# ShittyWizard/DiplomJourney

Measured on NVIDIA B200. Metric: candidate rollouts/s (MPC inner loop), higher is better.
Workload: dtype f32

## Files before the change

diplomjourney_b200/csrc/mpcb_handle.cuh:

```cuda
#pragma once
#include <string>
#include <vector>

#include "mpcb_types.cuh"

namespace mpcb {

struct DevBuf {
    void *p = nullptr;
    size_t cap = 0;
    cudaError_t ensure(size_t bytes) {
        if (bytes <= cap) return cudaSuccess;
        if (p) cudaFree(p);
        p = nullptr; cap = 0;
        size_t want = bytes + bytes / 4 + 256;
        cudaError_t e = cudaMalloc(&p, want);
        if (e == cudaSuccess) cap = want;
        return e;
    }
    void release() { if (p) cudaFree(p); p = nullptr; cap = 0; }
    template <typename T> T *as() { return reinterpret_cast<T *>(p); }
};

constexpr unsigned long long kSegCap = 1ULL << 22;
constexpr unsigned long long kTileBatch = 1ULL << 23;
constexpr unsigned long long kWideReduceSegs = 1ULL << 15;
constexpr unsigned long long kFrontierCap = 1ULL << 22;

}

struct mpcb_handle_s {
    int device = 0, sms = 148;
    cudaStream_t stream = nullptr;
    std::string err;
    bool have_grid = false, tables_ready = false;
    std::vector<double> hv, hb;
    double L = 0, delta_t = 0, v_min = 0, v_slow = 0;
    mpcb::GridTables g{};
    mpcb::DevBuf tab64, tab32, vtab, tab64_slow, vtab_slow, beta, leaf32, leaf32p, leaf32r, ctl32, ctl32_slow;
    mpcb::RowPairs row_ab{};
    double tol_scale = 1.0;
    int algo = MPCB_ALGO_AUTO;
    int refine = 1;
    int small_path = 1;
    int zero_copy = 1;
    int dump_direct = 0;
    int npt = 2;
    unsigned long long frontier_cap = mpcb::kFrontierCap;
    int subtree_cut = 2;
    int screen = 2;
    int prefilter = 1;
    int prune = 1;
    mpcb::DevBuf sp, segmin, worklist, misc, tau, bestJ, bestIdx, lock, ub, tile_list, reduce_scratch;
    mpcb::DevBuf in_state, in_target, in_origin, in_thr, in_flags, out_cost, out_index, out_traj, out_ctl, dump_rec, dump_j;
    mpcb::DevBuf cand, cand_J, cand_sel;
    mpcb::DevBuf node_list;
    unsigned node_cap = 1u << 15;
    unsigned cand_cap = 1u << 20;
    bool cand_auto = true;
    mpcb::DevBuf nccl_scratch;
    mpcb::DevBuf loop_log, loop_ticks, loop_status, loop_events, loop_final, loop_rng, loop_keys, small_in, small_out, fl_last, fl_k, fl_have, fl_flags, fl_count;
    void *pin_in = nullptr, *pin_out = nullptr;
    size_t pin_in_cap = 0, pin_out_cap = 0;
    mpcb_stats stats{};
};
```

diplomjourney_b200/csrc/mpcb_kernels.cu:

```cuda
#include <type_traits>

#include "mpcb_types.cuh"
#include "mpcb_bounds.cuh"
#include "mpcb_exact.cuh"

#ifndef MPCB_UNROLL2
#define MPCB_UNROLL2 8
#endif
#ifndef MPCB_UNROLL4
#define MPCB_UNROLL4 2
#endif
#ifndef MPCB_PN_CTA2
#define MPCB_PN_CTA2 512
#endif
#ifndef MPCB_UNROLL_ROWS
#define MPCB_UNROLL_ROWS 4
#endif
#ifndef MPCB_UNROLL_DIST
#define MPCB_UNROLL_DIST 7
#endif
#ifndef MPCB_UNROLL
#define MPCB_UNROLL 8
#endif

// ... 134 lines not shown
        walk_step_t<float>(t.x, t.y, t.z, t.w, xi, eta, psi, cp, sp);
    });
    return node_prefilter32(pf, xi, eta, psi, cp, sp) > __double2float_ru(bound + 8.0 * P.tol1);
}

__device__ __forceinline__ double node_lower_bound(const LaunchArgs &a, const SolveParams &P, const NodeFrame &f) {
    return lower_bound_from(a, P, f.u, f.w, f.Dp, f.nu, f.nw, 1.0, 0.0, f.ep, f.hp, f.base0, 1);
}

__device__ __forceinline__ double node_regs(const LaunchArgs &a, const NodeFrame &f, ParentRegs &pr, bool &near,
                                            double *base_direct) {
    pr.u = (float)f.u; pr.w = (float)f.w;
    pr.u2 = (float)(-2.0 * f.u); pr.w2 = (float)(-2.0 * f.w);
    const double dp_rem = split_distance(f.Dp, pr);
    pr.nu = (float)f.nu; pr.nw = (float)f.nw;
    pr.e2 = (float)(2.0 * f.ep); pr.h2 = (float)(2.0 * f.hp);
    near = !(f.Dp >= 4.0 * a.g.smax);
    if (base_direct) {
        pr.eh = 0.5f * pr.e2; pr.nhh = -0.5f * pr.h2;
        pr.u2s = (float)(-2.0 * kWd * kWd * f.u); pr.w2s = (float)(-2.0 * kWd * kWd * f.w);
        pr.D2s = (float)(kWd * kWd * (f.Dp * f.Dp));
        *base_direct = f.base0 - kWd * f.Dp - (double)pr.eh * (double)pr.eh - (double)pr.nhh * (double)pr.nhh;
    }
    return f.base0 + (near ? dp_rem : 0.0);
}

__device__ __forceinline__ double parent_setup(const LaunchArgs &a, const SolveParams &P,
                                               unsigned long long p, ParentRegs &pr, bool &near, bool &unmoved,
                                               double *lower_bound = nullptr, double *base_direct = nullptr) {
    NodeFrame f;
    node_frame(a, P, p, f);
    unmoved = f.unmoved;
    if (lower_bound) *lower_bound = node_lower_bound(a, P, f);
    return node_regs(a, f, pr, near, base_direct);
}

__device__ __forceinline__ bool cand_push(const LaunchArgs &a, long long n, long long j, double jrel) {
    if (!a.cand) return false;
    const unsigned slot = atomicAdd(a.cand_count, 1u);
    if (slot >= a.cand_cap) return false;
    Candidate c;
    c.j = j; c.jrel = jrel; c.n = (int)n; c.pad = 0;
    a.cand[slot] = c;
    return true;
}

__device__ __forceinline__ void take_candidate(const LaunchArgs &a, const SolveParams &P, long long n, long long j,
                                               double jrel32, double &bJ, long long &bj) {
    atomicAdd(a.counters + 1, 1ULL);
    if (cand_push(a, n, j, jrel32)) return;
    double J = a.refine ? exact_cost(a, P, j, nullptr, nullptr) : (P.Kbase + jrel32);
    lex_min(bJ, bj, J, j);
}

__device__ __forceinline__ void publish_best(const LaunchArgs &a, long long n, double bJ, long long bj,
                                             double *s_J, long long *s_j) {
    const int lane = threadIdx.x & 31, warp = threadIdx.x >> 5;
#pragma unroll
    for (int o = 16; o > 0; o >>= 1) {
        double oJ = __shfl_xor_sync(0xffffffffu, bJ, o);
        long long oj = __shfl_xor_sync(0xffffffffu, bj, o);
        lex_min(bJ, bj, oJ, oj);
    }
    if (lane == 0) { s_J[warp] = bJ; s_j[warp] = bj; }
    __syncthreads();
    if (threadIdx.x == 0) {
        for (int i = 1; i < kThreads / 32; ++i) lex_min(bJ, bj, s_J[i], s_j[i]);
        if (bj >= 0) {
            while (atomicCAS(a.lock + n, 0, 1) != 0) {}
            __threadfence();
            double cJ = *(volatile double *)(a.bestJ + n);
            long long cj = *(volatile long long *)(a.bestIdx + n);
            lex_min(cJ, cj, bJ, bj);
            *(volatile double *)(a.bestJ + n) = cJ;
            *(volatile long long *)(a.bestIdx + n) = cj;
            __threadfence();
            atomicExch(a.lock + n, 0);
        }
    }
    __syncthreads();
}

__device__ __forceinline__ void publish_segmin(const LaunchArgs &a, unsigned seg, double v) {
    v = warp_min(v);
    if ((threadIdx.x & 31) == 0 && v < INFINITY)
        atomicMin(reinterpret_cast<unsigned long long *>(a.segmin) + seg, ordered_key(v));
}

__device__ __forceinline__ void publish_segmin_lanes(const LaunchArgs &a, unsigned seg, double v) {
    const unsigned live = __ballot_sync(0xffffffffu, v < INFINITY);
    if (!live) return;
    const unsigned seg0 = __shfl_sync(0xffffffffu, seg, __ffs(live) - 1);
    if (__all_sync(0xffffffffu, !(v < INFINITY) || seg == seg0)) publish_segmin(a, seg0, v);
    else if (v < INFINITY) atomicMin(reinterpret_cast<unsigned long long *>(a.segmin) + seg, ordered_key(v));
}

__device__ __forceinline__ bool gate_closed(const LaunchArgs &a) {
    return a.gate != 0 && *(volatile const unsigned *)a.q_overflow != 0;
}

template <int PASS>
__device__ __forceinline__ void decode_work(const LaunchArgs &a, unsigned long long w, unsigned &seg,
                                            long long &n, unsigned long long &tile_lo, unsigned long long &tile_hi) {
    const unsigned sps = (unsigned)a.segs_per_solve;
    unsigned long long off;
    if (PASS == 1) { seg = (unsigned)w; off = 0; }
    else {
        unsigned long long e = a.tps == 1 ? w : w / a.tps;
        seg = a.worklist[e];
        off = w - e * a.tps;
    }
    unsigned nn = seg / sps;
    unsigned sidx = seg - nn * sps;
    n = nn;
    tile_lo = (unsigned long long)sidx * a.tps + off;
    tile_hi = tile_lo + (PASS == 1 ? a.tps : 1);
    if (tile_hi > a.tiles_per_solve) tile_hi = a.tiles_per_solve;
}

template <bool HEAD>
__device__ __forceinline__ float prefix_min_loop_far2(const float4 *__restrict__ tab, int npairs, const ParentRegs &pr,
                                                      float best) {
    const float2 U2 = make_float2(pr.u2s, pr.u2s), W2 = make_float2(pr.w2s, pr.w2s);
    const float2 D2 = make_float2(pr.D2s, pr.D2s), K2 = make_float2(kWd2f, kWd2f);
    const float2 NU = make_float2(pr.nu, pr.nu), NW = make_float2(pr.nw, pr.nw);
    const float2 EH = make_float2(pr.eh, pr.eh), NHH = make_float2(pr.nhh, pr.nhh);
    constexpr int kUnroll = MPCB_UNROLL;
#pragma unroll kUnroll
    for (int m = 0; m < npairs; ++m) {
        const float4 t0 = tab[2 * m], t1 = tab[2 * m + 1];
        const float2 A = make_float2(t0.x, t0.y), B = make_float2(t0.z, t0.w);
        const float2 R = make_float2(t1.x, t1.y), G = make_float2(t1.z, t1.w);
        const float2 dd = __ffma2_rn(U2, A, __ffma2_rn(W2, B, __ffma2_rn(K2, R, D2)));
        const float2 q = __ffma2_rn(NU, A, __ffma2_rn(NW, B, EH));
        float2 acc = __ffma2_rn(q, q, make_float2(sqrt_approx(dd.x), sqrt_approx(dd.y)));
        if (HEAD) { const float2 gg = __fadd2_rn(G, NHH); acc = __ffma2_rn(gg, gg, acc); }
        best = fminf(best, fminf(acc.x, acc.y));
    }
    return best;
}

template <bool HEAD>
__device__ __forceinline__ float prefix_min_loop_far2_lanes(const float4 *__restrict__ tab, int npairs, float u2s, float w2s,
                                                            float D2s, float nu, float nw, float eh, float nhh, int lane) {
    const float2 U2 = make_float2(u2s, u2s), W2 = make_float2(w2s, w2s), D2 = make_float2(D2s, D2s);
    const float2 K2 = make_float2(kWd2f, kWd2f), NU = make_float2(nu, nu), NW = make_float2(nw, nw);
    const float2 EH = make_float2(eh, eh), NHH = make_float2(nhh, nhh);
    float best = INFINITY;
    for (int m = lane; m < npairs; m += 32) {
        const float4 t0 = tab[2 * m], t1 = tab[2 * m + 1];
        const float2 A = make_float2(t0.x, t0.y), B = make_float2(t0.z, t0.w);
        const float2 R = make_float2(t1.x, t1.y), G = make_float2(t1.z, t1.w);
        const float2 dd = __ffma2_rn(U2, A, __ffma2_rn(W2, B, __ffma2_rn(K2, R, D2)));
        const float2 q = __ffma2_rn(NU, A, __ffma2_rn(NW, B, EH));
        float2 acc = __ffma2_rn(q, q, make_float2(sqrt_approx(dd.x), sqrt_approx(dd.y)));
        if (HEAD) { const float2 gg = __fadd2_rn(G, NHH); acc = __ffma2_rn(gg, gg, acc); }
        best = fminf(best, fminf(acc.x, acc.y));
    }
    return best;
}

template <bool HEAD, int NPT>
__device__ __forceinline__ void prefix_min_loop_far2xN(const float4 *__restrict__ tab, int npairs,
                                                       const ParentRegs (&p)[NPT], float (&best)[NPT]) {
    float2 U[NPT], W[NPT], D[NPT], NU[NPT], NW[NPT], E[NPT], Hh[NPT];
    float b[NPT];
// ... 34 lines not shown
#pragma unroll
    for (int k = 0; k < NPT; ++k) {
        U[k] = make_float2(-p[k].u2s, -p[k].u2s); W[k] = make_float2(-p[k].w2s, -p[k].w2s);
        D[k] = make_float2(-p[k].D2s, -p[k].D2s);
        NU[k] = make_float2(p[k].nu, p[k].nu); NW[k] = make_float2(p[k].nw, p[k].nw);
        E[k] = make_float2(p[k].eh, p[k].eh); Hh[k] = make_float2(p[k].nhh, p[k].nhh);
        C[k] = make_float2(cn[k], cn[k]);
        m[k] = -INFINITY;
    }
    const float2 K2 = make_float2(-kWd2f, -kWd2f);
    constexpr int kUnroll = NPT == 2 ? MPCB_UNROLL2 : MPCB_UNROLL4;
#pragma unroll kUnroll
    for (int i = 0; i < npairs; ++i) {
        const float4 t0 = tab[2 * i], t1 = tab[2 * i + 1];
        const float2 A = make_float2(t0.x, t0.y), B = make_float2(t0.z, t0.w);
        const float2 R = make_float2(t1.x, t1.y), G = make_float2(t1.z, t1.w);
#pragma unroll
        for (int k = 0; k < NPT; ++k) {
            const float2 ndd = __ffma2_rn(U[k], A, __ffma2_rn(W[k], B, __ffma2_rn(K2, R, D[k])));
            const float2 q = __ffma2_rn(NU[k], A, __ffma2_rn(NW[k], B, E[k]));
            float2 t = __ffma2_rn(make_float2(-q.x, -q.y), q, C[k]);
            if (HEAD) { const float2 gg = __fadd2_rn(G, Hh[k]); t = __ffma2_rn(make_float2(-gg.x, -gg.y), gg, t); }
            const float2 df = __ffma2_rn(t, t, ndd);
            m[k] = fmaxf(m[k], fmaxf(df.x, df.y));
        }
    }
#pragma unroll
    for (int k = 0; k < NPT; ++k) mx[k] = m[k];
}

template <bool HEAD, int NPT>
__device__ __forceinline__ void prefix_screen_loop_rows(const float4 *__restrict__ tab, int nv, int ppr,
                                                        const ParentRegs (&p)[NPT], const float (&cn)[NPT],
                                                        float (&mx)[NPT]) {
    float2 U[NPT], W[NPT], NU[NPT], NW[NPT], E[NPT], Hh[NPT], C[NPT];
    float nD[NPT], m[NPT];
#pragma unroll
    for (int k = 0; k < NPT; ++k) {
        U[k] = make_float2(-p[k].u2s, -p[k].u2s); W[k] = make_float2(-p[k].w2s, -p[k].w2s);
        nD[k] = -p[k].D2s;
        NU[k] = make_float2(p[k].nu, p[k].nu); NW[k] = make_float2(p[k].nw, p[k].nw);
        E[k] = make_float2(p[k].eh, p[k].eh); Hh[k] = make_float2(p[k].nhh, p[k].nhh);
        C[k] = make_float2(cn[k], cn[k]);
        m[k] = -INFINITY;
    }
    constexpr int kUnroll = NPT == 2 ? MPCB_UNROLL_ROWS : MPCB_UNROLL4;
    for (int iv = 0; iv < nv; ++iv) {
        const float4 *__restrict__ row = tab + 2 * iv * ppr;
        const float rv = row[1].x;
        float2 DV[NPT];
#pragma unroll
        for (int k = 0; k < NPT; ++k) { const float d = __fmaf_rn(-kWd2f, rv, nD[k]); DV[k] = make_float2(d, d); }
#pragma unroll kUnroll
        for (int i = 0; i < ppr; ++i) {
            const float4 t0 = row[2 * i];
            const float2 G = reinterpret_cast<const float2 *>(row + 2 * i + 1)[1];
            const float2 A = make_float2(t0.x, t0.y), B = make_float2(t0.z, t0.w);
#pragma unroll
            for (int k = 0; k < NPT; ++k) {
                const float2 ndd = __ffma2_rn(U[k], A, __ffma2_rn(W[k], B, DV[k]));
                const float2 q = __ffma2_rn(NU[k], A, __ffma2_rn(NW[k], B, E[k]));
                float2 t = __ffma2_rn(make_float2(-q.x, -q.y), q, C[k]);
                if (HEAD) { const float2 gg = __fadd2_rn(G, Hh[k]); t = __ffma2_rn(make_float2(-gg.x, -gg.y), gg, t); }
                const float2 df = __ffma2_rn(t, t, ndd);
                m[k] = fmaxf(m[k], fmaxf(df.x, df.y));
            }
        }
    }
#pragma unroll
    for (int k = 0; k < NPT; ++k) mx[k] = m[k];
}

template <int NPT>
__device__ __forceinline__ void prefix_dist_loop_rows(const RowPairs &ab, const float4 *__restrict__ tab, int nv, int ppr,
                                                      const ParentRegs (&p)[NPT], float (&mx)[NPT]) {
    float2 U[NPT], W[NPT];
    float nD[NPT], m[NPT];
#pragma unroll
    for (int k = 0; k < NPT; ++k) {
        U[k] = make_float2(-p[k].u2s, -p[k].u2s); W[k] = make_float2(-p[k].w2s, -p[k].w2s);
        nD[k] = -p[k].D2s;
        m[k] = -INFINITY;
    }
    constexpr int kUnroll = NPT == 2 ? MPCB_UNROLL_DIST : MPCB_UNROLL4;
    const float4 *__restrict__ row = tab;
    const float4 *pair = ab.ab;
    for (int iv = 0; iv < nv; ++iv, row += 2 * ppr, pair += ppr) {
        const float rv = row[1].x;
        float2 DV[NPT];
#pragma unroll
        for (int k = 0; k < NPT; ++k) { const float d = __fmaf_rn(-kWd2f, rv, nD[k]); DV[k] = make_float2(d, d); }
#pragma unroll kUnroll
        for (int i = 0; i < ppr; ++i) {
            const float4 t0 = pair[i];
            const float2 A = make_float2(t0.x, t0.y), B = make_float2(t0.z, t0.w);
#pragma unroll
            for (int k = 0; k < NPT; ++k) {
                const float2 ndd = __ffma2_rn(U[k], A, __ffma2_rn(W[k], B, DV[k]));
                m[k] = fmaxf(m[k], fmaxf(ndd.x, ndd.y));
            }
        }
    }
#pragma unroll
    for (int k = 0; k < NPT; ++k) mx[k] = m[k];
}

template <bool HEAD>
__device__ __forceinline__ float prefix_min_loop_scalar(const float4 *__restrict__ tab, int npairs, const ParentRegs &pr,
                                                        bool near, bool special, float Lspecial, float best) {
    for (int m = 0; m < npairs; ++m) {
        const float4 t0 = tab[2 * m], t1 = tab[2 * m + 1];
        float L0 = near ? leaf_val<HEAD, true>(t0.x, t0.z, t1.x, t1.z, pr) : leaf_val<HEAD, false>(t0.x, t0.z, t1.x, t1.z, pr);
        float L1 = near ? leaf_val<HEAD, true>(t0.y, t0.w, t1.y, t1.w, pr) : leaf_val<HEAD, false>(t0.y, t0.w, t1.y, t1.w, pr);
        if (special && t1.x == 0.f) L0 = Lspecial;
        if (special && t1.y == 0.f) L1 = Lspecial;
        best = fminf(best, fminf(L0, L1));
    }
    return best;
}

template <int PASS, bool HEAD, bool PRUNE = false, bool QMODE = false>
__global__ void __launch_bounds__((PASS == 1 && !PRUNE) ? kPrefixCta : kThreads, (PASS == 1 && !PRUNE) ? 1 : 4)
prefix_kernel(const LaunchArgs a) {
    static_assert(PASS == 1, "pass 2 of the prefix algorithm is refine_prefix_kernel");
    extern __shared__ float4 s_leaf[];
    const int tid = threadIdx.x;
    const int S = a.g.S;
    const bool single = S <= kLeafChunk;
    const float4 *__restrict__ gtab = PASS == 1 ? a.g.leaf32p : a.g.leaf32;
    auto chunk_f4 = [&](int cn) { return PASS == 1 ? 2 * ((cn + 1) >> 1) : cn; };
    if (single) {
        for (int i = tid; i < chunk_f4(S); i += blockDim.x) s_leaf[i] = __ldg(gtab + i);
        __syncthreads();
    }
    const unsigned groups = blockDim.x / kThreads;
    const unsigned long long qps = (a.tiles_per_solve + groups - 1) / groups;
    constexpr bool qmode = PASS == 1 && PRUNE && QMODE;
    const bool listed = PASS == 1 && PRUNE && !QMODE && a.tile_list != nullptr;
    if (PASS == 1 && PRUNE && gate_closed(a)) return;
    const unsigned qrounds = (unsigned)((S + kThreads - 1) / kThreads);
    if (qmode && blockIdx.x == 0 && tid == 0) atomicAdd(a.counters + 2, a.counters[3]);
    const unsigned long long nwork =
        qmode ? (unsigned long long)min(*a.q_count, a.q_cap) * qrounds
        : listed ? (unsigned long long)(*a.tile_count)
                 : PASS == 1 ? (unsigned long long)a.N * qps : (unsigned long long)(*a.work_count) * a.tps;
    unsigned long long cut_acc = 0;
    for (unsigned long long w = blockIdx.x; w < nwork; w += gridDim.x) {
        unsigned seg; long long n; unsigned long long tile_lo, tile_hi;
        unsigned long long p_q = 0; bool in_q = false;
        if (qmode) {
            const unsigned long long e = w / qrounds;
            const unsigned c = (unsigned)(w - e * qrounds) * kThreads + tid;
            const unsigned long long g = a.q_list[e];
            n = (long long)a.fd[1].div(g);
            p_q = (g - (unsigned long long)n * a.fd[1].d) * (unsigned long long)S + c;
            in_q = c < (unsigned)S;
            tile_lo = in_q ? (p_q - a.u_begin) / kThreads : 0;
            tile_hi = tile_lo + 1;
            seg = (unsigned)((unsigned long long)n * a.segs_per_solve + (a.tps == 1 ? tile_lo : tile_lo / a.tps));
        } else if (listed) {
            const unsigned long long g = a.tile_list[w];
            n = (long long)a.fd_tiles.div(g);
            tile_lo = g - (unsigned long long)n * a.tiles_per_solve;
            tile_hi = tile_lo + 1;
            seg = (unsigned)((unsigned long long)n * a.segs_per_solve + (a.tps == 1 ? tile_lo : tile_lo / a.tps));
        } else if (PASS == 1) {
            n = (long long)(w / qps);
// ... 249 lines not shown
            q.D2 = __shfl_sync(0xffffffffu, pr.D2, src); q.Dp = __shfl_sync(0xffffffffu, pr.Dp, src);
            q.nu = __shfl_sync(0xffffffffu, pr.nu, src); q.nw = __shfl_sync(0xffffffffu, pr.nw, src);
            q.e2 = __shfl_sync(0xffffffffu, pr.e2, src); q.h2 = __shfl_sync(0xffffffffu, pr.h2, src);
            const bool qnear = __shfl_sync(0xffffffffu, (int)near, src) != 0;
            const bool qspecial = __shfl_sync(0xffffffffu, (int)special, src) != 0;
            const float qLsp = __shfl_sync(0xffffffffu, Lspecial, src), qthr = __shfl_sync(0xffffffffu, thr, src);
            const double qbase = __shfl_sync(0xffffffffu, base, src);
            const unsigned long long qp = __shfl_sync(0xffffffffu, p, src);
            scan_node<HEAD>(a, P, tab, S, lane, q, qnear, qspecial, qLsp, qthr, qbase, qp, n, bJ, bj, cand_acc);
        }
        if (__any_sync(0xffffffffu, bj >= 0)) publish_best_warp(a, n, bJ, bj);
    }
    if (lane == 0 && seg_acc) atomicAdd(a.counters, seg_acc);
    flush_cand_count(a, cand_acc);
}

template <bool HEAD>
__global__ void __launch_bounds__(kThreads, 4) refine_scan_kernel(const LaunchArgs a) {
    extern __shared__ float4 s_leaf[];
    const int tid = threadIdx.x, lane = tid & 31;
    const int S = a.g.S;
    const bool single = S <= kLeafChunk;
    const unsigned count = min(*a.node_count, a.node_cap);
    if (count == 0) return;
    if (single) {
        for (int i = tid; i < S; i += blockDim.x) s_leaf[i] = __ldg(a.g.leaf32 + i);
        __syncthreads();
    }
    const float4 *__restrict__ tab = single ? s_leaf : a.g.leaf32;
    constexpr unsigned wpc = kThreads / 32;
    const unsigned warps = gridDim.x * wpc, wid = blockIdx.x * wpc + (tid >> 5);
    const unsigned per = (count + warps - 1) / warps;
    const unsigned i0 = min(count, wid * per), i1 = min(count, i0 + per);
    unsigned long long cand_acc = 0;
    long long cur_n = -1;
    double bJ = INFINITY; long long bj = -1;
    for (unsigned i = i0; i < i1; ++i) {
        const RefineNode e = a.node_list[i];
        if (e.n < 0) continue;
        if (e.n != cur_n) {
            if (__any_sync(0xffffffffu, bj >= 0)) publish_best_warp(a, cur_n, bJ, bj);
            cur_n = e.n; bJ = INFINITY; bj = -1;
        }
        ParentRegs q = {};
        q.u = e.u; q.w = e.w; q.u2 = e.u2; q.w2 = e.w2; q.D2 = e.D2; q.Dp = e.Dp; q.nu = e.nu; q.nw = e.nw;
        q.e2 = e.e2; q.h2 = e.h2;
        scan_node<HEAD>(a, a.sp[e.n], tab, S, lane, q, (e.flags & 1u) != 0, (e.flags & 2u) != 0, e.Lspecial, e.thr, e.base,
                        e.p, e.n, bJ, bj, cand_acc);
    }
    if (__any_sync(0xffffffffu, bj >= 0)) publish_best_warp(a, cur_n, bJ, bj);
    flush_cand_count(a, cand_acc);
}

__host__ __device__ constexpr int prefixn_cta(int npt) { return npt == 2 ? MPCB_PN_CTA2 : kPrefixCta / npt; }

static_assert(sizeof(LaunchArgs) + sizeof(RowPairs) <= 32764, "prefixn_kernel's parameters exceed the launch limit");

template <bool HEAD, int NPT, int SCREEN = 0>
__global__ void __launch_bounds__(prefixn_cta(NPT), NPT / 2)
prefixn_kernel(const LaunchArgs a, const __grid_constant__ RowPairs ab) {
    extern __shared__ float4 s_leaf[];
    constexpr int kCta = prefixn_cta(NPT);
    const int tid = threadIdx.x;
    const int S = a.g.S;
    const bool rows = SCREEN && a.g.ppr > 0;
    const bool single = rows || S <= kLeafChunk;
    const float4 *__restrict__ gtab = rows ? a.g.leaf32r : a.g.leaf32p;
    auto chunk_f4 = [&](int cn) { return 2 * ((cn + 1) >> 1); };
    if (single) {
        for (int i = tid; i < (rows ? 2 * a.g.nv * a.g.ppr : chunk_f4(S)); i += blockDim.x) s_leaf[i] = __ldg(gtab + i);
        __syncthreads();
    }
    constexpr unsigned groups = kCta * NPT / kThreads;
    static_assert(kCta * NPT % kThreads == 0, "a work item is a whole number of tiles");
    const unsigned long long qps = (a.tiles_per_solve + groups - 1) / groups;
    const unsigned long long nwork = (unsigned long long)a.N * qps;
    unsigned long long stage2_acc = 0;
    for (unsigned long long w = blockIdx.x; w < nwork; w += gridDim.x) {
        const long long n = (long long)(w / qps);
        const unsigned long long tile0 = (w - (unsigned long long)n * qps) * groups;
        const SolveParams &P = a.sp[n];
        if (__reduce_or_sync(0xffffffffu, (unsigned)P.flags & kFlagSkip)) continue;
        const bool origin_case = (P.flags & kFlagStartIsOrigin) != 0;
        ParentRegs pr[NPT] = {};
        bool near[NPT], special[NPT], active[NPT];
        double base[NPT];
        float best[NPT], Lspecial[NPT], cn[NPT];
        unsigned seg[NPT];
        bool all = true;
        double ubw = INFINITY;
        if (SCREEN) ubw = ordered_value(*(volatile unsigned long long *)(a.ub + n)) + P.tol1;
#pragma unroll
        for (int k = 0; k < NPT; ++k) {
            const unsigned node = tid + k * kCta;
            const unsigned long long tile = tile0 + node / kThreads;
            const unsigned long long p = a.u_begin + tile * kThreads + (node % kThreads);
            active[k] = tile < a.tiles_per_solve && p < a.u_end;
            seg[k] = (unsigned)((unsigned long long)n * a.segs_per_solve + (a.tps == 1 ? tile : tile / a.tps));
            bool unmoved = false;
            near[k] = false; base[k] = 0.0; best[k] = INFINITY;
            double base_direct = 0.0;
            if (active[k]) base[k] = parent_setup(a, P, p, pr[k], near[k], unmoved, nullptr, &base_direct);
            special[k] = active[k] && origin_case && unmoved;
            if (!(near[k] || special[k])) base[k] = base_direct;
            Lspecial[k] = (float)(P.special - 0.25 * (double)pr[k].e2 * (double)pr[k].e2);
            cn[k] = SCREEN ? __double2float_ru(ubw - base_direct) : 0.f;
            all = all && active[k] && !near[k] && !special[k];
        }
        bool hit[NPT];
#pragma unroll
        for (int k = 0; k < NPT; ++k) hit[k] = false;
        for (int c0 = 0; c0 < S; c0 += kLeafChunk) {
            const int cn_ = min(kLeafChunk, S - c0);
            if (!single) {
                __syncthreads();
                for (int i = tid; i < chunk_f4(cn_); i += blockDim.x) s_leaf[i] = __ldg(gtab + c0 + i);
                __syncthreads();
            }
            const int npairs = rows ? a.g.nv * a.g.ppr : (cn_ + 1) >> 1;
            if (all && SCREEN) {
                bool stage2 = true;
                if (SCREEN == 2 && rows) {
                    float mdd[NPT];
                    prefix_dist_loop_rows<NPT>(ab, s_leaf, a.g.nv, a.g.ppr, pr, mdd);
                    stage2 = false;
#pragma unroll
                    for (int k = 0; k < NPT; ++k) {
                        const float tmax = screen_stage1_tmax(a.g.sbox, HEAD, cn[k], pr[k].nu, pr[k].nw, pr[k].eh, pr[k].nhh);
                        const bool pass = screen_stage1_pass(tmax, mdd[k]);
                        stage2 = stage2 || pass;
                        stage2_acc += pass ? 1u : 0u;
                    }
                }
                if (stage2) {
                    float mx[NPT];
                    if (rows) prefix_screen_loop_rows<HEAD, NPT>(s_leaf, a.g.nv, a.g.ppr, pr, cn, mx);
                    else prefix_screen_loop_far2xN<HEAD, NPT>(s_leaf, npairs, pr, cn, mx);
#pragma unroll
                    for (int k = 0; k < NPT; ++k)
                        if (mx[k] > 0.f) { best[k] = prefix_min_loop_far2<HEAD>(s_leaf, npairs, pr[k], best[k]); hit[k] = true; }
                }
            } else if (all) {
                prefix_min_loop_far2xN<HEAD, NPT>(s_leaf, npairs, pr, best);
            } else {
#pragma unroll
                for (int k = 0; k < NPT; ++k) {
                    if (!active[k]) continue;
                    best[k] = (near[k] || special[k])
                                  ? prefix_min_loop_scalar<HEAD>(s_leaf, npairs, pr[k], near[k], special[k], Lspecial[k], best[k])
                                  : prefix_min_loop_far2<HEAD>(s_leaf, npairs, pr[k], best[k]);
                }
            }
        }
        if (SCREEN) {
            double v = INFINITY;
#pragma unroll
            for (int k = 0; k < NPT; ++k) if (hit[k]) v = fmin(v, base[k] + (double)best[k]);
            if (__any_sync(0xffffffffu, v < INFINITY)) {
                v = warp_min(v);
                if ((tid & 31) == 0) atomicMin(a.ub + n, ordered_key(v + 0.5 * P.tol1));
            }
        }
#pragma unroll
        for (int k = 0; k < NPT; ++k) {
            const double v = active[k] ? base[k] + (double)best[k] : INFINITY;
            publish_segmin(a, seg[k], (!SCREEN || v <= ubw) ? v : INFINITY);
        }
    }
    if (SCREEN == 2) {
#pragma unroll
        for (int o = 16; o > 0; o >>= 1) stage2_acc += __shfl_xor_sync(0xffffffffu, stage2_acc, o);
        if ((tid & 31) == 0 && stage2_acc) atomicAdd(a.counters + 7, stage2_acc);
    }
}

__global__ void __launch_bounds__(kThreads) frontier_expand_kernel(const LaunchArgs a, int k,
                                                                   const unsigned long long *__restrict__ src,
                                                                   const unsigned *src_count,
                                                                   unsigned long long *__restrict__ dst,
                                                                   unsigned *dst_count, unsigned *overflow) {
    if (*(volatile unsigned *)overflow) return;
    const unsigned long long S = (unsigned long long)a.g.S;
    const unsigned long long nsrc = src ? (unsigned long long)min(*src_count, a.q_cap) : (unsigned long long)a.N;
    const unsigned long long c_lo = src ? 0ULL : (unsigned long long)a.i0_begin;
    const unsigned long long nchild = src ? S : (unsigned long long)(a.i0_end - a.i0_begin);
    const unsigned long long total = nsrc * nchild;
    const FastDiv64 fdn = a.fd[a.H - 2 - k];
    const int steps = a.H - (k + 1);
    const unsigned long long below = a.fd[k + 1].d;
    const unsigned lane = threadIdx.x & 31u;
    unsigned long long cut = 0;
    for (unsigned long long t0 = blockIdx.x * (unsigned long long)kThreads + (threadIdx.x & ~31u); t0 < total;
         t0 += (unsigned long long)gridDim.x * kThreads) {
        const unsigned long long t = t0 + lane;
        bool keep = false;
        unsigned long long child = 0;
        if (t < total) {
            const unsigned long long e = t / nchild;
            child = (src ? src[e] : e) * S + (t - e * nchild + c_lo);
            const unsigned long long n = fdn.div(child);
            const SolveParams &P = a.sp[n];
            if (!(P.flags & kFlagSkip)) {
                unsigned long long rem = child - n * fdn.d;
                double xi = 0.0, eta = 0.0, psi = 0.0, cp = 1.0, sp = 0.0;
                for (int m = 0; m <= k; ++m) {
                    const FastDiv64 &fd = a.fd[a.H - 1 - k + m];
                    const unsigned long long i = fd.div(rem);
                    rem -= i * fd.d;
                    walk_step(ldg_d4(a.g.tab64 + i), xi, eta, psi, cp, sp);
                }
                const double bound = ordered_value(*(volatile unsigned long long *)(a.ub + n)) + P.tol1 + P.tol;
                keep = !(subtree_lower_bound(a, P, xi, eta, psi, cp, sp, steps) > bound);
                if (!keep) cut += below;
            }
        }
        const unsigned mk = __ballot_sync(0xffffffffu, keep);
        if (mk) {
            unsigned base = 0;
            if (lane == 0) base = atomicAdd(dst_count, (unsigned)__popc(mk));
            base = __shfl_sync(0xffffffffu, base, 0);
            const unsigned slot = base + __popc(mk & ((1u << lane) - 1u));
            if (keep) {
                if (slot < a.q_cap) dst[slot] = child;
                else *overflow = 1u;
            }
        }
    }
    for (int o = 16; o > 0; o >>= 1) cut += __shfl_xor_sync(0xffffffffu, cut, o);
    if (lane == 0 && cut) atomicAdd(a.counters + 3, cut);
}

__device__ __forceinline__ bool tile_survives(const LaunchArgs &a, unsigned long long g, unsigned &cut_nodes) {
    const unsigned long long n = a.fd_tiles.div(g), tile = g - n * a.tiles_per_solve;
    const SolveParams &P = a.sp[n];
    cut_nodes = 0;
    if (P.flags & kFlagSkip) return false;
    const unsigned long long p_lo = a.u_begin + tile * kThreads;
    const unsigned long long p_hi = min(p_lo + (unsigned long long)kThreads, a.u_end);
    const double bound = ordered_value(*(volatile unsigned long long *)(a.ub + n)) + P.tol1 + P.tol;
    bool keep = false;
    const unsigned long long q_hi = a.fd_S.div(p_hi - 1);
    for (unsigned long long q = a.fd_S.div(p_lo); q <= q_hi && !keep; ++q) {
        if (a.prefilter) {
            const Prefilter32 pf = prefilter32(a, P);
            float xi = 0.f, eta = 0.f, psi = 0.f, cp = 1.f, sp = 0.f;
            parent_digits(a, q, [&](unsigned i) {
                const float4 t = __ldg(a.g.tab32 + i);
                walk_step_t<float>(t.x, t.y, t.z, t.w, xi, eta, psi, cp, sp);
            });
// ... 674 lines not shown

__global__ void split_ub_min_kernel(const LaunchArgs a, const unsigned long long *all, int nranks) {
    const long long n = blockIdx.x * (long long)blockDim.x + threadIdx.x;
    if (n >= a.N) return;
    unsigned long long k = a.ub[n];
    for (int r = 0; r < nranks; ++r) k = min(k, all[(size_t)r * a.N + n]);
    a.ub[n] = k;
}

cudaError_t launch_split_ub_min(cudaStream_t st, const LaunchArgs &a, const unsigned long long *all, int nranks) {
    split_ub_min_kernel<<<(unsigned)((a.N + 127) / 128), 128, 0, st>>>(a, all, nranks);
    return cudaGetLastError();
}

cudaError_t launch_split_pack(cudaStream_t st, const LaunchArgs &a, SplitRec *mine) {
    split_pack_kernel<<<(unsigned)((a.N + 127) / 128), 128, 0, st>>>(a, mine);
    return cudaGetLastError();
}

cudaError_t launch_split_pick(cudaStream_t st, const LaunchArgs &a, const SplitRec *all, int nranks) {
    split_pick_kernel<<<(unsigned)((a.N + 127) / 128), 128, 0, st>>>(a, all, nranks);
    return cudaGetLastError();
}

static inline int grid_for(unsigned long long work, int sms, int per_sm) {
    unsigned long long cap = (unsigned long long)sms * per_sm;
    return (int)(work < cap ? (work ? work : 1) : cap);
}

cudaError_t launch_prep(cudaStream_t st, long long N, const double *state, const double *target,
                        const double *origin, const double *threshold, const uint8_t *flags, int cost_kind, int H,
                        int prefix, double smax, double dphimax, double tol_scale, SolveParams *out) {
    const int bs = 128;
    prep_kernel<<<(unsigned)((N + bs - 1) / bs), bs, 0, st>>>(N, state, target, origin, threshold, flags, cost_kind,
                                                            H, prefix, smax, dphimax, tol_scale, out);
    return cudaGetLastError();
}

static size_t prefix_smem(const LaunchArgs &a) {
    const size_t rows = 2 * (size_t)a.g.nv * a.g.ppr;
    const size_t flat = (size_t)(a.g.S < kLeafChunk ? a.g.S + 1 : kLeafChunk);
    return sizeof(float4) * (rows > flat ? rows : flat);
}

template <typename K>
static int resident_ctas(K kernel, size_t smem, int threads) {
    int n = 0;
    if (cudaOccupancyMaxActiveBlocksPerMultiprocessor(&n, kernel, threads, smem) != cudaSuccess || n < 1) n = 1;
    return n;
}

template <typename K>
static cudaError_t launch_persistent(K kernel, const LaunchArgs &a, int pass, size_t smem, int sms, cudaStream_t st,
                                     int threads = kThreads, const RowPairs *ab = nullptr) {
    if (smem > 48 * 1024) cudaFuncSetAttribute(kernel, cudaFuncAttributeMaxDynamicSharedMemorySize, (int)smem);
    const int slots = sms * resident_ctas(kernel, smem, threads);
    const int grid = pass == 1 ? (int)(a.total_segs < (unsigned long long)slots ? a.total_segs : slots) : slots;
    if constexpr (std::is_invocable_v<K, const LaunchArgs, const RowPairs>) kernel<<<grid, threads, smem, st>>>(a, *ab);
    else kernel<<<grid, threads, smem, st>>>(a);
    return cudaGetLastError();
}

cudaError_t launch_pass(cudaStream_t st, const LaunchArgs &a, const RowPairs &ab, int pass, bool prefix, int sms) {
    const bool head = a.cost_kind == 0;
    if (prefix) {
        const size_t sm = prefix_smem(a);
        if (pass == 1 && a.prune && a.g.S > kLeafChunk) {
            const size_t smq = sizeof(QEntry) * kWarpQueue * (kThreads / 32);
            if (a.q_list)
                return head ? launch_persistent(prefix_pruned_kernel<true, true>, a, pass, smq, sms, st)
                            : launch_persistent(prefix_pruned_kernel<false, true>, a, pass, smq, sms, st);
            return head ? launch_persistent(prefix_pruned_kernel<true>, a, pass, smq, sms, st)
                        : launch_persistent(prefix_pruned_kernel<false>, a, pass, smq, sms, st);
        }
        if (pass == 1 && a.prune && a.q_list)
            return head ? launch_persistent(prefix_kernel<1, true, true, true>, a, pass, sm, sms, st)
                        : launch_persistent(prefix_kernel<1, false, true, true>, a, pass, sm, sms, st);
        if (pass == 1 && a.prune)
            return head ? launch_persistent(prefix_kernel<1, true, true>, a, pass, sm, sms, st)
                        : launch_persistent(prefix_kernel<1, false, true>, a, pass, sm, sms, st);
#define MPCB_PN(NPT_, SCR_)                                                                                      \
    (head ? launch_persistent(prefixn_kernel<true, NPT_, SCR_>, a, pass, sm, sms, st, prefixn_cta(NPT_), &ab)    \
          : launch_persistent(prefixn_kernel<false, NPT_, SCR_>, a, pass, sm, sms, st, prefixn_cta(NPT_), &ab))
        if (pass == 1 && a.npt == 4) return a.screen == 2 ? MPCB_PN(4, 2) : a.screen ? MPCB_PN(4, 1) : MPCB_PN(4, 0);
        if (pass == 1 && a.npt == 2) return a.screen == 2 ? MPCB_PN(2, 2) : a.screen ? MPCB_PN(2, 1) : MPCB_PN(2, 0);
#undef MPCB_PN
        if (pass == 1)
            return head ? launch_persistent(prefix_kernel<1, true>, a, pass, sm, sms, st, kPrefixCta)
                        : launch_persistent(prefix_kernel<1, false>, a, pass, sm, sms, st, kPrefixCta);
        const size_t sm2 = sizeof(float4) * (size_t)(a.g.S <= kLeafChunk ? a.g.S : 0);
        return head ? launch_persistent(refine_prefix_kernel<true>, a, pass, sm2, sms, st)
                    : launch_persistent(refine_prefix_kernel<false>, a, pass, sm2, sms, st);
    }
    const int kind = a.mode == 1 ? 2 : (a.idx32 ? 1 : 0);
    const size_t lw_sm = (a.mode != 1 && a.lw_smem) ? sizeof(float2) * (size_t)a.g.S : 0;
#define MPCB_LW(P_, H_, K_) launch_persistent(leafwalk_kernel<P_, H_, K_>, a, pass, lw_sm, sms, st)
#define MPCB_LW_KIND(P_, H_) (kind == 2 ? MPCB_LW(P_, H_, 2) : kind == 1 ? MPCB_LW(P_, H_, 1) : MPCB_LW(P_, H_, 0))
    if (pass == 1) return head ? MPCB_LW_KIND(1, true) : MPCB_LW_KIND(1, false);
    return head ? MPCB_LW_KIND(2, true) : MPCB_LW_KIND(2, false);
#undef MPCB_LW_KIND
#undef MPCB_LW
}

cudaError_t launch_frontier_expand(cudaStream_t st, const LaunchArgs &a, int k, const unsigned long long *src,
                                   const unsigned *src_count, unsigned long long *dst, unsigned *dst_count,
                                   unsigned *overflow, int sms) {
    frontier_expand_kernel<<<sms * 8, kThreads, 0, st>>>(a, k, src, src_count, dst, dst_count, overflow);
    return cudaGetLastError();
}

cudaError_t launch_tilecut(cudaStream_t st, const LaunchArgs &a, unsigned long long g_begin, unsigned long long g_end,
                           unsigned long long *list, unsigned *count, unsigned long long list_cap) {
    if (g_end - g_begin > list_cap) return cudaErrorInvalidValue;
    const unsigned long long blocks = (g_end - g_begin + kThreads - 1) / kThreads;
    tilecut_kernel<<<(unsigned)blocks, kThreads, 0, st>>>(a, g_begin, g_end, list, count, list_cap);
    return cudaGetLastError();
}

cudaError_t launch_tilewalk_fallback(cudaStream_t st, const LaunchArgs &a, unsigned long long all_tiles, int sms) {
    const size_t sm = prefix_smem(a);
    const bool head = a.cost_kind == 0;
    auto go = [&](auto kernel) {
        const int grid = sms * resident_ctas(kernel, sm, kThreads);
        kernel<<<grid, kThreads, sm, st>>>(a, all_tiles);
        return cudaGetLastError();
    };
    return head ? go(tilewalk_fallback_kernel<true>) : go(tilewalk_fallback_kernel<false>);
}

cudaError_t launch_probe(cudaStream_t st, const LaunchArgs &a, int sms) {
    probe_kernel<<<grid_for((unsigned long long)a.N, sms, 8), kThreads, 0, st>>>(a);
    return cudaGetLastError();
}

cudaError_t launch_reduce_compact(cudaStream_t st, const LaunchArgs &a, double *tau, unsigned *worklist,
                                  unsigned *work_count, int sms) {
    reduce_compact_kernel<<<grid_for((unsigned long long)a.N, sms, 8), kThreads, 0, st>>>(a, tau, worklist,
                                                                                         work_count);
    return cudaGetLastError();
}

cudaError_t launch_reduce_compact_wide(cudaStream_t st, const LaunchArgs &a, double *tau, unsigned *worklist,
                                       unsigned *work_count, void *scratch, int sms, int *launches) {
    unsigned long long *solve_key = static_cast<unsigned long long *>(scratch);
    double *tau1 = reinterpret_cast<double *>(solve_key + a.N);
    cudaError_t e = cudaMemsetAsync(solve_key, 0xFF, sizeof(unsigned long long) * a.N, st);
    if (e != cudaSuccess) return e;
    const unsigned long long chunks = (unsigned long long)a.N * ((a.segs_per_solve + kReduceChunk - 1) / kReduceChunk);
    const int grid = grid_for(chunks, sms, 8);
    segmin_fold_kernel<<<grid, kThreads, 0, st>>>(a, solve_key);
    window_edge_kernel<<<(unsigned)((a.N + 127) / 128), 128, 0, st>>>(a, solve_key, tau, tau1);
    seg_compact_kernel<<<grid, kThreads, 0, st>>>(a, tau1, worklist, work_count);
    *launches += 3;
    return cudaGetLastError();
}

cudaError_t launch_refine_scan(cudaStream_t st, const LaunchArgs &a, int sms) {
    const size_t sm2 = sizeof(float4) * (size_t)(a.g.S <= kLeafChunk ? a.g.S : 0);
    return a.cost_kind == 0 ? launch_persistent(refine_scan_kernel<true>, a, 2, sm2, sms, st)
                            : launch_persistent(refine_scan_kernel<false>, a, 2, sm2, sms, st);
}

cudaError_t launch_cand_resolve(cudaStream_t st, const LaunchArgs &a, int sms) {
    cand_eval_kernel<<<sms * 4, kThreads, 0, st>>>(a);
    cand_select_kernel<<<sms * 4, kThreads, 0, st>>>(a);
    cand_merge_kernel<<<(unsigned)((a.N + 127) / 128), 128, 0, st>>>(a);
    return cudaGetLastError();
}
// ... 26 lines not shown
```

Before: 7996 billion.

## Restructure two-stage screen to keep only distance state and recompute rare survivors

In the SCREEN==2 path, each thread now keeps only the three distance fields per parent for the stage-1 bound, then recomputes the full parent setup serially for the few slots that pass the screen or need the direct path. This lowers register pressure, which is likely what allows the default of four parents per thread instead of two. It also raises the unroll for the NPT=4 distance loop, adds an early exit in publish_segmin when no lane in the warp holds a value, and falls back from screen mode 2 to 1 when there are no row pairs. The cost is repeating parent_setup for the survivors, and the stage-2 work becomes serial and divergent.

Result: faster. 9497 billion (median of 6 runs) (+18.8%).

```diff
diff --git a/diplomjourney_b200/csrc/mpcb_handle.cuh b/diplomjourney_b200/csrc/mpcb_handle.cuh
--- a/diplomjourney_b200/csrc/mpcb_handle.cuh
+++ b/diplomjourney_b200/csrc/mpcb_handle.cuh
@@ -45,7 +45,7 @@
     int small_path = 1;
     int zero_copy = 1;
     int dump_direct = 0;
-    int npt = 2;
+    int npt = 4;
     unsigned long long frontier_cap = mpcb::kFrontierCap;
     int subtree_cut = 2;
     int screen = 2;
diff --git a/diplomjourney_b200/csrc/mpcb_kernels.cu b/diplomjourney_b200/csrc/mpcb_kernels.cu
--- a/diplomjourney_b200/csrc/mpcb_kernels.cu
+++ b/diplomjourney_b200/csrc/mpcb_kernels.cu
@@ -240,6 +240,7 @@
 }
 
 __device__ __forceinline__ void publish_segmin(const LaunchArgs &a, unsigned seg, double v) {
+    if (!__any_sync(0xffffffffu, v < INFINITY)) return;
     v = warp_min(v);
     if ((threadIdx.x & 31) == 0 && v < INFINITY)
         atomicMin(reinterpret_cast<unsigned long long *>(a.segmin) + seg, ordered_key(v));
@@ -440,7 +441,7 @@
         nD[k] = -p[k].D2s;
         m[k] = -INFINITY;
     }
-    constexpr int kUnroll = NPT == 2 ? MPCB_UNROLL_DIST : MPCB_UNROLL4;
+    constexpr int kUnroll = MPCB_UNROLL_DIST;
     const float4 *__restrict__ row = tab;
     const float4 *pair = ab.ab;
     for (int iv = 0; iv < nv; ++iv, row += 2 * ppr, pair += ppr) {
@@ -856,89 +857,144 @@
         const SolveParams &P = a.sp[n];
         if (__reduce_or_sync(0xffffffffu, (unsigned)P.flags & kFlagSkip)) continue;
         const bool origin_case = (P.flags & kFlagStartIsOrigin) != 0;
-        ParentRegs pr[NPT] = {};
-        bool near[NPT], special[NPT], active[NPT];
-        double base[NPT];
-        float best[NPT], Lspecial[NPT], cn[NPT];
-        unsigned seg[NPT];
-        bool all = true;
+        auto slot = [&](int k, unsigned long long &p, unsigned &sg) {
+            const unsigned node = tid + k * kCta;
+            const unsigned long long tile = tile0 + node / kThreads;
+            p = a.u_begin + tile * kThreads + (node % kThreads);
+            sg = (unsigned)((unsigned long long)n * a.segs_per_solve + (a.tps == 1 ? tile : tile / a.tps));
+            return tile < a.tiles_per_solve && p < a.u_end;
+        };
         double ubw = INFINITY;
         if (SCREEN) ubw = ordered_value(*(volatile unsigned long long *)(a.ub + n)) + P.tol1;
-#pragma unroll
-        for (int k = 0; k < NPT; ++k) {
-            const unsigned node = tid + k * kCta;
-            const unsigned long long tile = tile0 + node / kThreads;
-            const unsigned long long p = a.u_begin + tile * kThreads + (node % kThreads);
-            active[k] = tile < a.tiles_per_solve && p < a.u_end;
-            seg[k] = (unsigned)((unsigned long long)n * a.segs_per_solve + (a.tps == 1 ? tile : tile / a.tps));
-            bool unmoved = false;
-            near[k] = false; base[k] = 0.0; best[k] = INFINITY;
-            double base_direct = 0.0;
-            if (active[k]) base[k] = parent_setup(a, P, p, pr[k], near[k], unmoved, nullptr, &base_direct);
-            special[k] = active[k] && origin_case && unmoved;
-            if (!(near[k] || special[k])) base[k] = base_direct;
-            Lspecial[k] = (float)(P.special - 0.25 * (double)pr[k].e2 * (double)pr[k].e2);
-            cn[k] = SCREEN ? __double2float_ru(ubw - base_direct) : 0.f;
-            all = all && active[k] && !near[k] && !special[k];
-        }
-        bool hit[NPT];
-#pragma unroll
-        for (int k = 0; k < NPT; ++k) hit[k] = false;
-        for (int c0 = 0; c0 < S; c0 += kLeafChunk) {
-            const int cn_ = min(kLeafChunk, S - c0);
-            if (!single) {
-                __syncthreads();
-                for (int i = tid; i < chunk_f4(cn_); i += blockDim.x) s_leaf[i] = __ldg(gtab + c0 + i);
-                __syncthreads();
+        const int npairs_rows = a.g.nv * a.g.ppr;
+        double v[NPT];
+        double vhit = INFINITY;
+#pragma unroll
+        for (int k = 0; k < NPT; ++k) v[k] = INFINITY;
+        if constexpr (SCREEN == 2) {
+            ParentRegs s1[NPT] = {};
+            float tmax[NPT];
+            unsigned staged = 0, direct = 0;
+#pragma unroll
+            for (int k = 0; k < NPT; ++k) {
+                unsigned long long p;
+                unsigned sg;
+                tmax[k] = 0.f;
+                if (!slot(k, p, sg)) continue;
+                ParentRegs q;
+                bool nr, um;
+                double bd;
+                parent_setup(a, P, p, q, nr, um, nullptr, &bd);
+                if (nr || (origin_case && um)) { direct |= 1u << k; continue; }
+                staged |= 1u << k;
+                s1[k].u2s = q.u2s; s1[k].w2s = q.w2s; s1[k].D2s = q.D2s;
+                tmax[k] = screen_stage1_tmax(a.g.sbox, HEAD, __double2float_ru(ubw - bd), q.nu, q.nw, q.eh, q.nhh);
             }
-            const int npairs = rows ? a.g.nv * a.g.ppr : (cn_ + 1) >> 1;
-            if (all && SCREEN) {
-                bool stage2 = true;
-                if (SCREEN == 2 && rows) {
-                    float mdd[NPT];
-                    prefix_dist_loop_rows<NPT>(ab, s_leaf, a.g.nv, a.g.ppr, pr, mdd);
-                    stage2 = false;
-#pragma unroll
-                    for (int k = 0; k < NPT; ++k) {
-                        const float tmax = screen_stage1_tmax(a.g.sbox, HEAD, cn[k], pr[k].nu, pr[k].nw, pr[k].eh, pr[k].nhh);
-                        const bool pass = screen_stage1_pass(tmax, mdd[k]);
-                        stage2 = stage2 || pass;
-                        stage2_acc += pass ? 1u : 0u;
+            unsigned rare = direct;
+            if (__reduce_or_sync(0xffffffffu, staged)) {
+                float mdd[NPT];
+                prefix_dist_loop_rows<NPT>(ab, s_leaf, a.g.nv, a.g.ppr, s1, mdd);
+#pragma unroll
+                for (int k = 0; k < NPT; ++k)
+                    if (((staged >> k) & 1u) && screen_stage1_pass(tmax[k], mdd[k])) { rare |= 1u << k; ++stage2_acc; }
+            }
+            for (unsigned m = rare; m; m &= m - 1) {
+                const int k = __ffs(m) - 1;
+                unsigned long long p;
+                unsigned sg;
+                slot(k, p, sg);
+                ParentRegs pr;
+                bool near, unmoved;
+                double bd;
+                double base = parent_setup(a, P, p, pr, near, unmoved, nullptr, &bd);
+                float best = INFINITY;
+                if ((direct >> k) & 1u) {
+                    const float Ls = (float)(P.special - 0.25 * (double)pr.e2 * (double)pr.e2);
+                    best = prefix_min_loop_scalar<HEAD>(s_leaf, npairs_rows, pr, near, origin_case && unmoved, Ls, best);
+                } else {
+                    base = bd;
+                    const ParentRegs one[1] = {pr};
+                    const float cn[1] = {__double2float_ru(ubw - bd)};
+                    float mx[1];
+                    prefix_screen_loop_rows<HEAD, 1>(s_leaf, a.g.nv, a.g.ppr, one, cn, mx);
+                    if (mx[0] > 0.f) {
+                        best = prefix_min_loop_far2<HEAD>(s_leaf, npairs_rows, pr, best);
+                        vhit = fmin(vhit, base + (double)best);
                     }
                 }
-                if (stage2) {
+#pragma unroll
+                for (int j = 0; j < NPT; ++j)
+                    if (j == k) v[j] = base + (double)best;
+            }
+        } else {
+            ParentRegs pr[NPT] = {};
+            bool near[NPT], special[NPT], active[NPT];
+            double base[NPT];
+            float best[NPT], Lspecial[NPT], cn[NPT];
+            bool all = true;
+#pragma unroll
+            for (int k = 0; k < NPT; ++k) {
+                unsigned long long p;
+                unsigned sg;
+                active[k] = slot(k, p, sg);
+                bool unmoved = false;
+                near[k] = false; base[k] = 0.0; best[k] = INFINITY;
+                double base_direct = 0.0;
+                if (active[k]) base[k] = parent_setup(a, P, p, pr[k], near[k], unmoved, nullptr, &base_direct);
+                special[k] = active[k] && origin_case && unmoved;
+                if (!(near[k] || special[k])) base[k] = base_direct;
+                Lspecial[k] = (float)(P.special - 0.25 * (double)pr[k].e2 * (double)pr[k].e2);
+                cn[k] = SCREEN ? __double2float_ru(ubw - base_direct) : 0.f;
+                all = all && active[k] && !near[k] && !special[k];
+            }
+            bool hit[NPT];
+#pragma unroll
+            for (int k = 0; k < NPT; ++k) hit[k] = false;
+            for (int c0 = 0; c0 < S; c0 += kLeafChunk) {
+                const int cn_ = min(kLeafChunk, S - c0);
+                if (!single) {
+                    __syncthreads();
+                    for (int i = tid; i < chunk_f4(cn_); i += blockDim.x) s_leaf[i] = __ldg(gtab + c0 + i);
+                    __syncthreads();
+                }
+                const int npairs = rows ? npairs_rows : (cn_ + 1) >> 1;
+                if (all && SCREEN) {
                     float mx[NPT];
                     if (rows) prefix_screen_loop_rows<HEAD, NPT>(s_leaf, a.g.nv, a.g.ppr, pr, cn, mx);
                     else prefix_screen_loop_far2xN<HEAD, NPT>(s_leaf, npairs, pr, cn, mx);
 #pragma unroll
                     for (int k = 0; k < NPT; ++k)
                         if (mx[k] > 0.f) { best[k] = prefix_min_loop_far2<HEAD>(s_leaf, npairs, pr[k], best[k]); hit[k] = true; }
-                }
-            } else if (all) {
-                prefix_min_loop_far2xN<HEAD, NPT>(s_leaf, npairs, pr, best);
-            } else {
-#pragma unroll
-                for (int k = 0; k < NPT; ++k) {
-                    if (!active[k]) continue;
-                    best[k] = (near[k] || special[k])
-                                  ? prefix_min_loop_scalar<HEAD>(s_leaf, npairs, pr[k], near[k], special[k], Lspecial[k], best[k])
-                                  : prefix_min_loop_far2<HEAD>(s_leaf, npairs, pr[k], best[k]);
+                } else if (all) {
+                    prefix_min_loop_far2xN<HEAD, NPT>(s_leaf, npairs, pr, best);
+                } else {
+#pragma unroll
+                    for (int k = 0; k < NPT; ++k) {
+                        if (!active[k]) continue;
+                        best[k] = (near[k] || special[k])
+                                      ? prefix_min_loop_scalar<HEAD>(s_leaf, npairs, pr[k], near[k], special[k], Lspecial[k], best[k])
+                                      : prefix_min_loop_far2<HEAD>(s_leaf, npairs, pr[k], best[k]);
+                    }
                 }
             }
+#pragma unroll
+            for (int k = 0; k < NPT; ++k) {
+                if (active[k]) v[k] = base[k] + (double)best[k];
+                if (hit[k]) vhit = fmin(vhit, v[k]);
+            }
         }
         if (SCREEN) {
-            double v = INFINITY;
-#pragma unroll
-            for (int k = 0; k < NPT; ++k) if (hit[k]) v = fmin(v, base[k] + (double)best[k]);
-            if (__any_sync(0xffffffffu, v < INFINITY)) {
-                v = warp_min(v);
-                if ((tid & 31) == 0) atomicMin(a.ub + n, ordered_key(v + 0.5 * P.tol1));
+            if (__any_sync(0xffffffffu, vhit < INFINITY)) {
+                vhit = warp_min(vhit);
+                if ((tid & 31) == 0) atomicMin(a.ub + n, ordered_key(vhit + 0.5 * P.tol1));
             }
         }
 #pragma unroll
         for (int k = 0; k < NPT; ++k) {
-            const double v = active[k] ? base[k] + (double)best[k] : INFINITY;
-            publish_segmin(a, seg[k], (!SCREEN || v <= ubw) ? v : INFINITY);
+            unsigned long long p;
+            unsigned sg;
+            slot(k, p, sg);
+            publish_segmin(a, sg, (!SCREEN || v[k] <= ubw) ? v[k] : INFINITY);
         }
     }
     if (SCREEN == 2) {
@@ -1779,8 +1835,9 @@
 #define MPCB_PN(NPT_, SCR_)                                                                                      \
     (head ? launch_persistent(prefixn_kernel<true, NPT_, SCR_>, a, pass, sm, sms, st, prefixn_cta(NPT_), &ab)    \
           : launch_persistent(prefixn_kernel<false, NPT_, SCR_>, a, pass, sm, sms, st, prefixn_cta(NPT_), &ab))
-        if (pass == 1 && a.npt == 4) return a.screen == 2 ? MPCB_PN(4, 2) : a.screen ? MPCB_PN(4, 1) : MPCB_PN(4, 0);
-        if (pass == 1 && a.npt == 2) return a.screen == 2 ? MPCB_PN(2, 2) : a.screen ? MPCB_PN(2, 1) : MPCB_PN(2, 0);
+        const int scr = a.screen == 2 && a.g.ppr == 0 ? 1 : a.screen;
+        if (pass == 1 && a.npt == 4) return scr == 2 ? MPCB_PN(4, 2) : scr ? MPCB_PN(4, 1) : MPCB_PN(4, 0);
+        if (pass == 1 && a.npt == 2) return scr == 2 ? MPCB_PN(2, 2) : scr ? MPCB_PN(2, 1) : MPCB_PN(2, 0);
 #undef MPCB_PN
         if (pass == 1)
             return head ? launch_persistent(prefix_kernel<1, true>, a, pass, sm, sms, st, kPrefixCta)
```
